# muzishen/IMAGDressing

Hardware: AMD Instinct MI355X
Metric: 512x512 50-step images/sec (whole node) (higher is better)
Workload: dtype bf16

## Files before the change

imagdressing_amd/_lib.py:

```python
from __future__ import annotations

import ctypes as C
import os

_HERE = os.path.dirname(os.path.abspath(__file__))
LIB_PATH = os.environ.get("IMD_LIB_PATH") or os.path.join(_HERE, "libimagdressing_hip.so")

ABI_VERSION = 9

u16p = C.POINTER(C.c_uint16)
f32p = C.POINTER(C.c_float)


class _Sized(C.Structure):

    def __init__(self, *args, **kw):
        super().__init__(*args, **kw)
        self.struct_bytes = C.sizeof(self)


class HeadsDest(C.Structure):
    _fields_ = [("ptr", C.c_void_p), ("kind", C.c_int), ("DP", C.c_int), ("L", C.c_int), ("scale", C.c_float)]


# ... 58 lines not shown
        ("z", C.c_void_p), ("eps", C.c_void_p), ("x_next", C.c_void_p),
        ("B", C.c_int), ("HW", C.c_int),
        ("guidance", C.c_float), ("sqrt_a_t", C.c_float), ("sqrt_1m_a_t", C.c_float),
        ("sqrt_a_prev", C.c_float), ("sqrt_1m_a_prev", C.c_float),
        ("mask", C.c_void_p), ("z_img", C.c_void_p), ("noise", C.c_void_p),
        ("sqrt_a_next", C.c_float), ("sqrt_1m_a_next", C.c_float), ("dtype", C.c_int),
        ("coefs", C.c_void_p), ("var_noise", C.c_void_p), ("sigma", C.c_float),
    ]


SYMBOLS = {
    "imd_abi_version": (C.c_int, []),
    "imd_last_error": (C.c_char_p, []),
    "imd_device_check": (C.c_int, [C.c_int]),
    "imd_conv_gemm": (C.c_int, [C.POINTER(ConvGemmParams), C.c_int, C.c_void_p]),
    "imd_conv_gemm_auto_cfg": (C.c_int, [C.c_int, C.c_int]),
    "imd_conv_gemm_auto_split": (C.c_int, [C.c_int, C.c_int, C.c_int, C.c_int]),
    "imd_attention": (C.c_int, [C.POINTER(AttnParams), C.c_void_p]),
    "imd_attention_dup_supported": (C.c_int, [C.c_int, C.c_int, C.c_int]),
    "imd_attention_phase_split_supported": (C.c_int, [C.c_int]),
    "imd_attention_fp8": (C.c_int, [C.POINTER(AttnParams), C.c_int, C.c_int, C.c_int, C.c_void_p]),
    "imd_attn_quantize_fp8": (C.c_int, [C.c_void_p, C.c_void_p, C.c_int, C.c_long, C.c_int, C.c_int, C.c_float, C.c_int, C.c_void_p]),
    "imd_set_tuning": (C.c_int, [C.c_int, C.c_int]),
    "imd_get_tuning": (C.c_int, [C.c_int]),
    "imd_attn_padded_dims": (C.c_int, [C.c_int, C.POINTER(C.c_int), C.POINTER(C.c_int)]),
    "imd_groupnorm": (C.c_int, [C.POINTER(GroupNormParams), C.c_void_p]),
    "imd_groupnorm_coeffs": (C.c_int, [C.POINTER(GroupNormParams), C.c_void_p, C.c_void_p, C.c_void_p]),
    "imd_conv_patch_supported": (C.c_int, [C.POINTER(ConvGemmParams)]),
    "imd_conv_patch2_supported": (C.c_int, [C.POINTER(ConvGemmParams)]),
    "imd_conv_patch3_supported": (C.c_int, [C.POINTER(ConvGemmParams)]),
# ... 56 lines not shown
```

imagdressing_amd/csrc/capi.cpp:

```cpp
#include <atomic>
#include <mutex>
#include <stdarg.h>
#include <stdio.h>
#include <string.h>

#include "imd_kernels.h"

namespace {
thread_local char g_err[512] = "";
}

int imd_set_error(const char* fmt, ...) {
    va_list ap;
    va_start(ap, fmt);
    vsnprintf(g_err, sizeof(g_err), fmt, ap);
    va_end(ap);
    return 1;
}

int imd_check_launch(const char* what) {
    hipError_t e = hipGetLastError();
    if (e != hipSuccess) return imd_set_error("%s: launch failed: %s", what, hipGetErrorString(e));
    return 0;
}
// ... 58 lines not shown
    IMD_REQUIRE(p != nullptr, "conv_gemm: null params");
    IMD_REQUIRE_SIZE(p, "conv_gemm");
    IMD_REQUIRE(p->x && p->w, "conv_gemm: null input/weight pointer");
    IMD_REQUIRE(p->mode == IMD_OUT_HEADS || p->out != nullptr, "conv_gemm: null output pointer");
    IMD_REQUIRE(p->Hout > 0 && p->Wout > 0 && p->Hin > 0 && p->Win > 0, "conv_gemm: bad geometry");
    IMD_REQUIRE(p->stride == 1 || p->stride == 2, "conv_gemm: stride must be 1 or 2");
    IMD_REQUIRE(p->M % (p->Hout * p->Wout) == 0, "conv_gemm: M (%d) is not a multiple of Hout*Wout (%d)", p->M, p->Hout * p->Wout);
    if (p->mode == IMD_OUT_HEADS) {
        IMD_REQUIRE(p->hC > 0 && p->hH > 0 && p->hD > 0 && p->hC == p->hH * p->hD, "conv_gemm: bad head split C=%d H=%d D=%d", p->hC, p->hH, p->hD);
        IMD_REQUIRE(p->N % p->hC == 0 && p->N / p->hC <= 3, "conv_gemm: N (%d) must be 1..3 splits of %d channels", p->N, p->hC);
        IMD_REQUIRE(p->hD % 8 == 0, "conv_gemm: head dim must be a multiple of 8");
        IMD_REQUIRE(p->act != IMD_ACT_GEGLU && !p->out_f32, "conv_gemm: head-split output excludes GEGLU / fp32 output");
    }
    if (p->act == IMD_ACT_GEGLU) IMD_REQUIRE(!p->out_f32 && !p->res, "conv_gemm: GEGLU excludes fp32 output and residual");
    return imd_launch_conv_gemm(*p, cfg, (hipStream_t)stream);
}

int imd_conv_gemm_auto_cfg(int M, int N) { return imd_conv_gemm_choose_cfg(M, N); }
int imd_conv_gemm_auto_split(int M, int N, int K, int cfg) { return imd_conv_gemm_choose_split(M, N, K, cfg < 0 ? imd_conv_gemm_choose_cfg(M, N) : cfg); }

int imd_attention(const imd_attn_params* p, void* stream) {
    IMD_REQUIRE(p != nullptr, "attention: null params");
    IMD_REQUIRE_SIZE(p, "attention");
    IMD_REQUIRE(p->q && p->k1 && p->v1t && p->out, "attention: null q/k/v/out pointer");
    IMD_REQUIRE((p->k2 == nullptr) == (p->v2t == nullptr), "attention: k2 and v2t must be given together");
    IMD_REQUIRE(p->out_ld >= p->H * p->D && p->out_ld % 4 == 0, "attention: bad out_ld %d", p->out_ld);
    return imd_launch_attention(*p, (hipStream_t)stream);
}

int imd_attention_fp8(const imd_attn_params* p, int eq, int ek, int ev, void* stream) {
// ... 193 lines not shown
```

imagdressing_amd/csrc/conv_gemm.hip:

```cpp
#include "gemm_common.h"

namespace {

template <int BM, int BN, int BK, int WAVES_M> struct TileCfg {
    static constexpr int STRIDE = BK * 2 + 16;
    static constexpr int MAIN = 2 * (BM + BN) * STRIDE;
    static constexpr int CLD = BN + 4;
    static constexpr int EROWS = BM / WAVES_M;
    static constexpr int EPI = EROWS * CLD * 4;
    static constexpr int LDS = MAIN > EPI ? MAIN : EPI;
};

template <bool F16, int BM, int BN, int BK, int WAVES_M, int WAVES_N, int DEPTH>
__global__ __launch_bounds__(WAVES_M * WAVES_N * 64, (WAVES_M * WAVES_N == 4) ? 2 : 1) void conv_gemm_kernel(const ConvGemmParams p) {
    constexpr int NT = WAVES_M * WAVES_N * 64;
    using E = El<F16>;
    using T = TileCfg<BM, BN, BK, WAVES_M>;
    constexpr int TM = BM / WAVES_M / 32;
    constexpr int TN = BN / WAVES_N / 32;
    constexpr int STRIDE = T::STRIDE;
    constexpr int VPR = BK / 8;
    constexpr int RSTEP = NT / VPR;
    constexpr int A_VECS = BM / RSTEP;
    constexpr int W_VECS = BN / RSTEP;
// ... 576 lines not shown
    if (s > 8) s = 8;
    return s < 1 ? 1 : (int)s;
}

bool imd_conv_gemm_fill_extents(ConvGemmParams& p) {
    if (p.Hout <= 0 || p.Wout <= 0 || p.M <= 0) return false;
    const size_t npix = (size_t)(p.M / (p.Hout * p.Wout)) * p.Hin * p.Win;
    if (npix == 0) return false;
    const size_t xb = ((npix - 1) * (size_t)p.x_pix_stride + p.Cin) * 2, wb = (size_t)p.N * p.K * 2;
    if (xb >= 0xffffffffull || wb >= 0xffffffffull) return false;
    p.x_bytes = (uint32_t)xb;
    p.w_bytes = (uint32_t)wb;
    return true;
}

int imd_launch_conv_gemm(const ConvGemmParams& p_in, int cfg, hipStream_t s) {
    ConvGemmParams p = p_in;
    if (p.M <= 0 || p.N <= 0 || p.K <= 0) return imd_set_error("conv_gemm: empty problem M=%d N=%d K=%d", p.M, p.N, p.K);
    if ((p.K % 8) || (p.Cin % 8) || (p.x_pix_stride % 8))
        return imd_set_error("conv_gemm: K (%d), Cin (%d) and pixel stride (%d) must be multiples of 8", p.K, p.Cin, p.x_pix_stride);
    if (p.N % 4) return imd_set_error("conv_gemm: N (%d) must be a multiple of 4", p.N);
    if (p.taps != 1 && p.taps != 9) return imd_set_error("conv_gemm: taps must be 1 or 9 (got %d)", p.taps);
    if (p.K != p.taps * p.Cin) return imd_set_error("conv_gemm: K (%d) != taps*Cin (%d)", p.K, p.taps * p.Cin);
    if (p.mode == OUT_HEADS && (p.hD % 8)) return imd_set_error("conv_gemm: head dim (%d) must be a multiple of 8", p.hD);
    if (p.act == ACT_GEGLU && (p.N % 8)) return imd_set_error("conv_gemm: GEGLU needs N %% 8 == 0");
    if (!imd_conv_gemm_fill_extents(p)) return imd_set_error("conv_gemm: operand larger than 4 GiB");
    if (cfg < 0) cfg = imd_conv_gemm_choose_cfg(p.M, p.N);
    if (p.split_k < 1) p.split_k = 1;
    const unsigned tag = (unsigned)p_in.flags & IMD_TUNING_TAG_MASK;
    if (tag != 0 && tag != (unsigned)IMD_TUNING_PER_CALL)
        return imd_set_error("conv_gemm: flags = 0x%x on entry is neither 0 nor IMD_TUNING_PER_CALL | bits (an uninitialised parameter block?)", (unsigned)p_in.flags);
// ... 31 lines not shown
                                      : (long)((p.M + bm - 1) / bm) * ((p.N + bn - 1) / bn);
        if (tiles > IMD_SPLITK_COUNTERS || (size_t)p.M * p.N * 4 >= 0x80000000ull) p.splitk_counters = nullptr;
    }
    if (p.split_k > 1) {
        if (p.mode == OUT_HEADS || p.act == ACT_GEGLU) return imd_set_error("conv_gemm: split-K supports row-major epilogues only");
        if (!p.splitk_ws) return imd_set_error("conv_gemm: split_k = %d needs a workspace", p.split_k);
    }
    if (p.dtype != IMD_DTYPE_BF16 && p.dtype != IMD_DTYPE_F16) return imd_set_error("conv_gemm: unknown dtype %d", p.dtype);
    if ((p.gn_a != nullptr) != (p.gn_b != nullptr)) return imd_set_error("conv_gemm: gn_a and gn_b must be given together");
    if (p.gn_a != nullptr && cfg != 5) return imd_set_error("conv_gemm: the fused GroupNorm prologue needs tile config 5 (got %d)", cfg);
    if (p.res_rows != 0 && cfg != 12)
        return imd_set_error("conv_gemm: a periodic residual (res_rows = %d) exists in the K = 320 row-resident projection only (tile config 12, got %d)", p.res_rows, cfg);
    if (p.gn_in_partial != nullptr && !imd_row_linear_gn_in_supported_of(p, cfg))
        return imd_set_error("conv_gemm: gn_in_* (GroupNorm of the input rows) exists in the row-resident projections only (tile configs 12 / 13 / 14 with H W a multiple of "
                             "their row block; got cfg=%d K=%d HW=%d): ask imd_row_linear_gn_in_supported() first", cfg, p.K, p.Hout * p.Wout);
    const bool h = p.dtype == IMD_DTYPE_F16;
    switch (cfg) {
        case 0: return h ? launch_cfg<true, 128, 128, 64, 2, 2>(p, s) : launch_cfg<false, 128, 128, 64, 2, 2>(p, s);
        case 1: return h ? launch_cfg<true, 128, 64, 64, 2, 2>(p, s) : launch_cfg<false, 128, 64, 64, 2, 2>(p, s);
        case 2: return h ? launch_cfg<true, 64, 64, 64, 2, 2>(p, s) : launch_cfg<false, 64, 64, 64, 2, 2>(p, s);
        case 3: return h ? launch_cfg<true, 64, 64, 64, 2, 2, 4>(p, s) : launch_cfg<false, 64, 64, 64, 2, 2, 4>(p, s);
        case 4: return h ? launch_cfg<true, 128, 128, 32, 2, 2>(p, s) : launch_cfg<false, 128, 128, 32, 2, 2>(p, s);
        case 6: return h ? launch_cfg<true, 64, 320, 32, 2, 2>(p, s) : launch_cfg<false, 64, 320, 32, 2, 2>(p, s);
        case 7: return h ? launch_cfg<true, 64, 64, 32, 2, 2, 4>(p, s) : launch_cfg<false, 64, 64, 32, 2, 2, 4>(p, s);
        case 8: return h ? launch_cfg<true, 128, 128, 32, 2, 2, 4>(p, s) : launch_cfg<false, 128, 128, 32, 2, 2, 4>(p, s);
        case 9: return h ? launch_cfg<true, 256, 128, 32, 4, 2>(p, s) : launch_cfg<false, 256, 128, 32, 4, 2>(p, s);
        case 10: return h ? launch_cfg<true, 256, 256, 32, 4, 2>(p, s) : launch_cfg<false, 256, 256, 32, 4, 2>(p, s);
        case 11: return h ? launch_cfg<true, 128, 320, 64, 4, 2>(p, s) : launch_cfg<false, 128, 320, 64, 4, 2>(p, s);
        case 5: {
            int rc = imd_launch_conv_patch(p, s);
            if (rc || p.split_k <= 1 || p.splitk_counters != nullptr) return rc;
            return launch_splitk_finish(p, s, "conv_patch split-K finish");
        }
        case 29: {
            p.splitk_counters = nullptr;
            int rc = imd_launch_conv_patch64(p, s);
            if (rc || p.split_k <= 1) return rc;
            return launch_splitk_finish(p, s, "conv_patch split-K finish");
        }
        case 21: {
            p.splitk_counters = nullptr;
            int rc = imd_launch_conv_patch2(p, s);
            if (rc || p.split_k <= 1) return rc;
            return launch_splitk_finish(p, s, "conv_patch2 split-K finish");
        }
// ... 42 lines not shown
```

imagdressing_amd/csrc/conv_patch.hip:

```cpp
#include <type_traits>

#include "gemm_common.h"
#include "lds_dma.h"

namespace {

constexpr int TH = 8, TW = 16;
constexpr int PW = TW + 2, PH = TH + 2;
constexpr int NPIX = PH * PW;
constexpr int CK = 32;
constexpr int RSTR = CK * 2 + 16;
constexpr int BN = 128;
constexpr int A_BYTES = NPIX * RSTR;
constexpr int W_BYTES = BN * RSTR;
constexpr int MAIN_LDS = 2 * A_BYTES + 2 * W_BYTES;
constexpr int CLD = BN + 4;
constexpr int EROWS = 64;
constexpr int EPI_LDS = EROWS * CLD * 4;
constexpr int PATCH_LDS = MAIN_LDS > EPI_LDS ? MAIN_LDS : EPI_LDS;
constexpr int A_VECS = (NPIX * (CK / 8) + 255) / 256;
__device__ constexpr unsigned char kColPix[32] = {0, 1, 2, 3, 8, 9, 10, 11, 12, 13, 14, 15, 4, 5, 6, 7,
                                                  30, 31, 16, 17, 22, 23, 24, 25, 26, 27, 28, 29, 18, 19, 20, 21};
constexpr int W_VECS = BN * (CK / 8) / 256;

// ... 1 lines not shown
constexpr int PATCH_DMA_LDS = 2 * AB_D + NWR_D * WB_D;
static_assert(PATCH_DMA_LDS >= EPI_LDS, "the epilogue tile must fit the main-loop LDS");
template <int CKD> struct PD {
    static constexpr int RB = CKD * 2, LPR = RB / 16;
    static constexpr int APIECES = (NPIX * RB + 1023) / 1024;
    static constexpr int APW = (APIECES + 3) / 4;
    static constexpr int AB = APW * 4 * 1024;
    static constexpr int WPW = BN * RB / 1024 / 4;
    static constexpr int WB = WPW * 4 * 1024;
    static constexpr int NWR = CKD == 32 ? 3 : 2;
    static constexpr int LDS = 2 * AB + NWR * WB;
    static_assert(LDS >= EPI_LDS, "the epilogue tile must fit the main-loop LDS");
    static __device__ __forceinline__ int swz(int r) { return CKD == 32 ? (r >> 2) & 3 : (r >> 1) & 7; }
};

template <bool F16, bool DMA, int CKD = 32>
__global__ __launch_bounds__(256, CKD == 32 ? 3 : 2) void conv3x3_patch_kernel(const ConvGemmParams p) {
    static_assert(CKD == 32 || DMA, "64-channel chunks exist for the LDS-DMA form only");
    using G = PD<CKD>;
    using E = El<F16>;
    extern __shared__ __attribute__((aligned(16))) char smem[];
    char* const Abuf = smem;
    char* const Wbuf = smem + 2 * A_BYTES;

    const int tid = threadIdx.x;
    const int lane = tid & 63;
    const int wave = tid >> 6;
    const int wm0 = (wave >> 1) * 64;
    const int wn0 = (wave & 1) * 64;
    const int hi = lane >> 5, col = lane & 31;
    const int cpix = kColPix[col];

    const int H = p.Hout, W = p.Wout;
// ... 98 lines not shown
#pragma unroll
            for (int r = 0; r < 16; ++r) acc[a][bb][r] = 0.f;

    int a_frag[2];
#pragma unroll
    for (int bb = 0; bb < 2; ++bb) {
        const int q = wm0 + bb * 32 + cpix;
        a_frag[bb] = ((q / TW) * PW + (q % TW)) * RSTR + hi * 16;
    }
    const int w_frag = (wn0 + col) * RSTR + hi * 16;
    const bool wave_live = n0 + wn0 < p.N;

    if constexpr (DMA) {
        const int wv = __builtin_amdgcn_readfirstlane(wave);
        const uint32_t smem_base = (uint32_t)(uintptr_t)smem;
        const v4i_t dx = raw_rsrc(p.x, p.x_bytes), dw = raw_rsrc(p.w, p.w_bytes);
        constexpr uint32_t FAR = 0x80000000u;
        uint32_t acur[G::APW], wcur[G::WPW];
        uint32_t adst[G::APW], wdst[G::WPW];
#pragma unroll
        for (int i = 0; i < G::APW; ++i) {
            const int slot = (wv * G::APW + i) * 64 + lane, pp = slot / G::LPR, piece = (slot % G::LPR) ^ G::swz(pp);
            acur[i] = FAR;
            if (pp < NPIX) {
                const int iy = y0 - 1 + pp / PW, ix = x0 - 1 + pp % PW;
                if ((unsigned)iy < (unsigned)H && (unsigned)ix < (unsigned)W) {
                    const int sy = p.ups ? (iy >> 1) : iy, sx = p.ups ? (ix >> 1) : ix;
                    acur[i] = (uint32_t)(((b * p.Hin + sy) * p.Win + sx) * p.x_pix_stride + piece * 8 + c_begin * CKD) * 2u;
                }
            }
            adst[i] = smem_base + (uint32_t)((wv * G::APW + i) * 1024);
        }
#pragma unroll
        for (int i = 0; i < G::WPW; ++i) {
            const int slot = (wv * G::WPW + i) * 64 + lane, row = slot / G::LPR, piece = (slot % G::LPR) ^ G::swz(row);
            wcur[i] = (n0 + row < p.N) ? (uint32_t)(((size_t)(n0 + row) * p.K + piece * 8 + c_begin * CKD) * 2) : FAR;
            wdst[i] = smem_base + (uint32_t)(2 * G::AB + (wv * G::WPW + i) * 1024);
        }
        const uint32_t w_tap = (uint32_t)(p.Cin * 2), w_chunk = (uint32_t)(CKD * 2) - 8u * w_tap;
        auto dma_patch = [&](auto buf_c) __attribute__((always_inline)) {
#pragma unroll
            for (int i = 0; i < G::APW; ++i) {
                asm volatile("s_add_u32 m0, %1, %3\n\ts_nop 0\n\tbuffer_load_dwordx4 %0, %2, 0 offen lds"
                             : : "v"(acur[i]), "s"(adst[i]), "s"(dx), "n"(decltype(buf_c)::value * G::AB) : "memory", "scc");
                acur[i] += (uint32_t)(CKD * 2);
            }
        };
        auto dma_w = [&](auto ring_c, auto cross_c) __attribute__((always_inline)) {
#pragma unroll
            for (int i = 0; i < G::WPW; ++i) {
                asm volatile("s_add_u32 m0, %1, %3\n\ts_nop 0\n\tbuffer_load_dwordx4 %0, %2, 0 offen lds"
                             : : "v"(wcur[i]), "s"(wdst[i]), "s"(dw), "n"(decltype(ring_c)::value * G::WB) : "memory", "scc");
                wcur[i] += decltype(cross_c)::value ? w_chunk : w_tap;
            }
// ... 253 lines not shown

bool imd_conv_patch_supported(const ConvGemmParams& p) {
    const bool geom = p.ups ? (p.Hout == 2 * p.Hin && p.Wout == 2 * p.Win && p.gn_a == nullptr && !(g_gemm_flags & 512))
                            : (p.Hin == p.Hout && p.Win == p.Wout);
    return p.taps == 9 && p.stride == 1 && !p.pad_br_only && geom && p.Hout >= TH && p.Wout >= TW && (p.Cin % CK) == 0 &&
           p.mode == OUT_ROWMAJOR && p.act != ACT_GEGLU;
}

bool imd_conv_patch64_supported(const ConvGemmParams& p) {
    return imd_conv_patch_supported(p) && (p.Cin % 64) == 0 && p.gn_a == nullptr && !(g_gemm_flags & 512) && p.x_bytes < 0x80000000u && p.w_bytes < 0x80000000u;
}

int imd_launch_conv_patch64(const ConvGemmParams& p, hipStream_t s) {
    if (!imd_conv_patch64_supported(p)) return imd_set_error("conv_patch (128-byte rows): unsupported problem (needs 3x3 stride 1, H >= 8, W >= 16, Cin %% 64 == 0, operands < 2 GiB, no fused GroupNorm)");
    const bool h = p.dtype == IMD_DTYPE_F16;
    typedef void (*kern_t)(const ConvGemmParams);
    const kern_t kern = h ? conv3x3_patch_kernel<true, true, 64> : conv3x3_patch_kernel<false, true, 64>;
    if (int rc_attr = imd_lds_attr(reinterpret_cast<const void*>(kern), PD<64>::LDS, "conv_patch")) return rc_attr;
    const int B = p.M / (p.Hout * p.Wout);
    const long blocks = (long)B * ((p.Hout + TH - 1) / TH) * ((p.Wout + TW - 1) / TW) * ((p.N + BN - 1) / BN);
    hipLaunchKernelGGL(kern, dim3((unsigned)blocks, (unsigned)p.split_k), dim3(256), PD<64>::LDS, s, p);
    return imd_check_launch("conv_patch (128-byte rows)");
}

int imd_launch_conv_patch(const ConvGemmParams& p, hipStream_t s) {
    if (!imd_conv_patch_supported(p)) return imd_set_error("conv_patch: unsupported geometry (needs 3x3 stride 1, H >= 8, W >= 16, Cin %% 32 == 0)");
    const bool h = p.dtype == IMD_DTYPE_F16;
    const bool dma = p.gn_a == nullptr && !(g_gemm_flags & 512) && (p.ups || (p.x_bytes < 0x80000000u && p.w_bytes < 0x80000000u));
    if (p.ups && (p.x_bytes >= 0x80000000u || p.w_bytes >= 0x80000000u)) return imd_set_error("conv_patch: fused upsample needs operands < 2 GiB");
    typedef void (*kern_t)(const ConvGemmParams);
    const kern_t kern = dma ? (h ? conv3x3_patch_kernel<true, true> : conv3x3_patch_kernel<false, true>)
                            : (h ? conv3x3_patch_kernel<true, false> : conv3x3_patch_kernel<false, false>);
    const int lds = dma ? PATCH_DMA_LDS : PATCH_LDS;
    if (int rc_attr = imd_lds_attr(reinterpret_cast<const void*>(kern), lds, "conv_patch")) return rc_attr;
    const int B = p.M / (p.Hout * p.Wout);
    const long blocks = (long)B * ((p.Hout + TH - 1) / TH) * ((p.Wout + TW - 1) / TW) * ((p.N + BN - 1) / BN);
    hipLaunchKernelGGL(kern, dim3((unsigned)blocks, (unsigned)p.split_k), dim3(256), lds, s, p);
    return imd_check_launch("conv_patch");
}
```

imagdressing_amd/csrc/imd_kernels.h:

```cpp
#pragma once
#include <hip/hip_runtime.h>
#include <stdint.h>

#include "../../include/imagdressing_hip.h"

typedef uint16_t bf16_t;
typedef imd_heads_dest HeadsDest;
typedef imd_conv_gemm_params ConvGemmParams;
typedef imd_attn_params AttnParams;
typedef imd_groupnorm_params GroupNormParams;
typedef imd_layernorm_params LayerNormParams;
typedef imd_ddim_params DdimParams;

enum { ACT_NONE = IMD_ACT_NONE, ACT_SILU = IMD_ACT_SILU, ACT_GEGLU = IMD_ACT_GEGLU, ACT_GELU = IMD_ACT_GELU, ACT_QUICK_GELU = IMD_ACT_QUICK_GELU };
enum { OUT_ROWMAJOR = IMD_OUT_ROWMAJOR, OUT_HEADS = IMD_OUT_HEADS };

int imd_set_error(const char* fmt, ...);
int imd_check_launch(const char* what);
int imd_lds_attr(const void* kern, int bytes, const char* what);
int imd_cu_count8();

int imd_conv_gemm_choose_cfg(int M, int N);
int imd_conv_gemm_choose_split(int M, int N, int K, int cfg);
int imd_launch_conv_gemm(const ConvGemmParams& p, int cfg, hipStream_t s);
bool imd_conv_gemm_fill_extents(ConvGemmParams& p);
bool imd_conv_patch_supported(const ConvGemmParams& p);
bool imd_conv_patch2_supported(const ConvGemmParams& p);
int imd_launch_conv_patch2(const ConvGemmParams& p, hipStream_t s);
bool imd_conv_patch3_supported(const ConvGemmParams& p);
int imd_launch_conv_patch3(const ConvGemmParams& p, hipStream_t s);
bool imd_conv_patch4_supported(const ConvGemmParams& p);
int imd_launch_conv_patch4(const ConvGemmParams& p, hipStream_t s);
int imd_conv_patch3_stats_parts_of(const ConvGemmParams& p, int nw);
bool imd_conv_patch64_supported(const ConvGemmParams& p);
int imd_launch_conv_patch64(const ConvGemmParams& p, hipStream_t s);
bool imd_conv_img_supported(const ConvGemmParams& p);
int imd_launch_conv_img(const ConvGemmParams& p, hipStream_t s);
int imd_conv_patch_stats_parts_of(const ConvGemmParams& p);
int imd_conv_gemm_stats_parts_of(const ConvGemmParams& p, int cfg);
bool imd_conv_gemm_gn_out_supported_of(const ConvGemmParams& p, int cfg);
bool imd_row_linear_gn_in_supported_of(const ConvGemmParams& p, int cfg);
int imd_launch_conv_patch(const ConvGemmParams& p, hipStream_t s);
bool imd_row_linear_supported(const ConvGemmParams& p);
int imd_launch_row_linear(const ConvGemmParams& p, int ln, float ln_eps, hipStream_t s);
bool imd_row_linear_k640_supported(const ConvGemmParams& p);
int imd_launch_row_linear_k640(const ConvGemmParams& p, int ln, float ln_eps, hipStream_t s);
bool imd_row_linear_k1280_supported(const ConvGemmParams& p);
int imd_launch_row_linear_k1280(const ConvGemmParams& p, int ln, float ln_eps, hipStream_t s);
bool imd_row_qkv_supported(const ConvGemmParams& p);
int imd_launch_row_qkv(const ConvGemmParams& p, int ln, float ln_eps, hipStream_t s);
bool imd_gemm_dma_supported(const ConvGemmParams& p);
int imd_launch_gemm_dma(const ConvGemmParams& p, hipStream_t s);
int imd_launch_gemm_dma128(const ConvGemmParams& p, int stages, hipStream_t s);
int imd_launch_gemm_dma256(const ConvGemmParams& p, int form, hipStream_t s);
bool imd_conv_dma_supported(const ConvGemmParams& p);
int imd_launch_ff_geglu(const imd_ff_params& p, hipStream_t s);
int imd_launch_attention(const AttnParams& p, hipStream_t s);
// ... 30 lines not shown
```

imagdressing_amd/ops.py:

```python
from __future__ import annotations

import functools
import ctypes as C
from typing import Dict, Optional, Sequence, Tuple

import torch

from . import _lib as L

ACT_NONE, ACT_SILU, ACT_GEGLU, ACT_GELU, ACT_QUICK_GELU = 0, 1, 2, 3, 4
bf16 = torch.bfloat16
f16 = torch.float16
DTYPE_CODE = {torch.bfloat16: 0, torch.float16: 1}


def _code(t: torch.Tensor, name: str = "tensor") -> int:
    try:
        return DTYPE_CODE[t.dtype]
    except KeyError:
        raise L.ImdError(f"{name}: expected a bfloat16 or float16 tensor, got {t.dtype}") from None


try:
    _raw_stream, _cur_dev = torch._C._cuda_getCurrentRawStream, torch._C._cuda_getDevice
# ... 12 lines not shown
        raise TypeError(f"{name}: expected a torch.Tensor, got {type(t)}")
    if not t.is_cuda:
        raise L.ImdError(f"{name}: tensor is on {t.device}; imagdressing_amd runs on MI355X only (no CPU path)")
    if t.dtype != dtype:
        raise L.ImdError(f"{name}: expected dtype {dtype}, got {t.dtype}")
    if not t.is_contiguous():
        raise L.ImdError(f"{name}: tensor must be contiguous")
    return t.data_ptr()


def _opt(t: Optional[torch.Tensor], dtype, name: str) -> Optional[int]:
    return None if t is None else _dev(t, dtype, name)


_checked_devices = set()


def ensure_device(device: torch.device):
    if device.type != "cuda":
        raise L.ImdError(f"tensor is on {device}; imagdressing_amd runs on MI355X (gfx950) only -- there is no CPU path")
    idx = device.index if device.index is not None else torch.cuda.current_device()
    if idx not in _checked_devices:
        L.check(L.load().imd_device_check(idx))
        _checked_devices.add(idx)


_ws: Dict[Tuple, torch.Tensor] = {}


def workspace(tag: str, shape: Sequence[int], dtype, device, init=None) -> torch.Tensor:
# ... 57 lines not shown
PATCH_CONV = True
PATCH_MIN_W = 32
SPLITK_IN_KERNEL = False
FUSED_FF = True
FUSED_FF_MIN_ROWS = 24576
import os as _os
FUSED_GN_STATS = _os.environ.get("IMD_FUSED_GN_STATS", "1") != "0"
CFG_PAIR_DEDUP = _os.environ.get("IMD_CFG_PAIR_DEDUP", "1") != "0"
FUSED_GN_CONV = _os.environ.get("IMD_FUSED_GN_CONV", "0") == "1"
FUSED_GN_FINISH = _os.environ.get("IMD_FUSED_GN_FINISH", "0") == "1"
FUSED_GN_PROJ = _os.environ.get("IMD_FUSED_GN_PROJ", "1") != "0"
FUSED_CONCAT_STATS = _os.environ.get("IMD_FUSED_CONCAT_STATS", "1") != "0"
PERIODIC_RES = _os.environ.get("IMD_PERIODIC_RES", "1") != "0"
GENERIC_GN_STATS = _os.environ.get("IMD_GENERIC_GN_STATS", "0") == "1"
TEMB_TABLE = _os.environ.get("IMD_TEMB_TABLE", "1") != "0"
FUSED_GN_PROJ_CFGS = tuple(int(c) for c in _os.environ.get("IMD_FUSED_GN_PROJ_CFGS", "12,13,14").split(",") if c)
CFG_PAIR_ATTN = _os.environ.get("IMD_CFG_PAIR_ATTN", "1") != "0"
FUSED_LN = True
GEMM_TRACE = None
GEMM_EVENT_HOOK = None
_GEMM_TABLE = None
_CFG_DECISIONS: Dict[Tuple, Tuple[int, int]] = {}

TUNING_PER_CALL = 0x5A000000
ATTN_VARIANT_MAX = 13


import contextvars

_TUNING = contextvars.ContextVar("imd_tuning_scope", default=None)
# ... 47 lines not shown
                _GEMM_TABLE = json.load(f).get("shapes", {})
        except FileNotFoundError:
            _GEMM_TABLE = {}
    return _GEMM_TABLE


def conv_gemm(
    x: torch.Tensor, w: torch.Tensor, *, M: int, N: int, Cin: int, taps: int = 1,
    Hin: int = 1, Win: int = 1, Hout: int = 1, Wout: int = 1, stride: int = 1, ups: bool = False,
    x_pix_stride: Optional[int] = None, out: Optional[torch.Tensor] = None, out_ld: Optional[int] = None,
    bias: Optional[torch.Tensor] = None, rowvec: Optional[torch.Tensor] = None, rowvec_stride: int = 0,
    rowvec_off: int = 0, res: Optional[torch.Tensor] = None, res_ld: Optional[int] = None, out_scale: float = 1.0,
    act: int = ACT_NONE, out_f32: bool = False,
    heads: Optional[dict] = None, cfg: int = -1, split_k: int = 0,
    gn: Optional[tuple] = None, pad_br_only: bool = False, ln_eps: Optional[float] = None, gn_stats_groups: int = 0,
    gn_out: Optional[tuple] = None, gn_in: Optional[tuple] = None,
) -> Optional[torch.Tensor]:
    ensure_device(x.device)
    K = taps * Cin
    p = L.ConvGemmParams()
    p.flags = _gemm_call_flags()
    dt = x.dtype
    p.dtype = _code(x, "x")
    p.x = _dev(x, dt, "x")
    p.w = _dev(w, dt, "w")
    if w.numel() != N * K:
        raise L.ImdError(f"conv_gemm: weight has {w.numel()} elements, expected N*K = {N}*{K}")
    p.M, p.N, p.K = M, N, K
    p.Cin, p.taps, p.Hin, p.Win, p.Hout, p.Wout, p.stride, p.ups = Cin, taps, Hin, Win, Hout, Wout, stride, int(ups)
    p.x_pix_stride = Cin if x_pix_stride is None else x_pix_stride
    p.bias = _opt(bias, torch.float32, "bias")
# ... 131 lines not shown
            out._imd_gn_applied = True
            return out
        p.gn_out_gamma = p.gn_out_beta = None
        p.gn_out_groups = 0
    stats = None
    if gn_stats_groups and FUSED_GN_STATS and heads is None and not out_f32 and act != ACT_GEGLU and \
            (cfg in (5, 22, 23, 29) or split_k > 1 or (GENERIC_GN_STATS and cfg in (-1, 0, 1, 2, 3, 4, 7))):
        p.gn_stats_groups = gn_stats_groups
        nparts = lib.imd_conv_gemm_stats_parts(C.byref(p), cfg)
        if nparts > 0:
            Bimg = M // (Hout * Wout)
            stats = (torch.empty((Bimg, nparts, gn_stats_groups, 2), dtype=torch.float32, device=x.device), nparts, gn_stats_groups)
            p.gn_stats_out = stats[0].data_ptr()
        else:
            p.gn_stats_groups = 0
    if GEMM_EVENT_HOOK is not None:
        e0, e1 = torch.cuda.Event(enable_timing=True), torch.cuda.Event(enable_timing=True)
        e0.record()
        L.check(lib.imd_conv_gemm(C.byref(p), cfg, _stream()))
        e1.record()
        GEMM_EVENT_HOOK.setdefault((f"{M},{N},{K},{taps},{stride},{int(ups)}|{Hout}x{Wout}", cfg, split_k), []).append((e0, e1))
    else:
        L.check(lib.imd_conv_gemm(C.byref(p), cfg, _stream()))
    if stats is not None:
        out._imd_gn_stats = stats
    return out


_splitk_ws: Dict[Tuple, torch.Tensor] = {}


_splitk_cnt: Dict[Tuple, torch.Tensor] = {}


def splitk_counters(device) -> torch.Tensor:
    key = (str(device), _stream())
    t = _splitk_cnt.get(key)
    if t is None:
# ... 55 lines not shown
    ensure_device(x2d.device)
    M, C_ = x2d.shape
    dt = x2d.dtype
    if out is None:
        out = torch.empty((M, C_), dtype=dt, device=x2d.device)
    p = L.FfParams()
    p.x, p.w1, p.b1 = _dev(x2d, dt, "x"), _dev(packed["w1"], dt, "w1"), _dev(packed["b1"], torch.float32, "b1")
    p.w2, p.b2, p.out = _dev(packed["w2"], dt, "w2"), _dev(packed["b2"], torch.float32, "b2"), _dev(out, dt, "out")
    p.M, p.C, p.inner, p.x_ld, p.out_ld = M, packed["C"], packed["inner"], x2d.stride(0), out.stride(0)
    p.ln, p.ln_eps, p.dtype = int(packed["ln"]), float(ln_eps), _code(x2d, "x")
    _count("gemm_conv", 2.0 * M * packed["C"] * 2 * packed["inner"] + 2.0 * M * packed["inner"] * packed["C"])
    L.check(L.load().imd_ff_geglu(C.byref(p), _stream()))
    return out


def conv2d_nhwc(x: torch.Tensor, w: torch.Tensor, bias=None, *, taps=9, stride=1, ups=False, rowvec=None,
                rowvec_stride=0, rowvec_off=0, res=None, out_scale=1.0, act=ACT_NONE, out_f32=False, cfg=-1, split_k=0, gn=None,
                pad_br_only=False, gn_stats_groups=0, gn_out=None, gn_in=None) -> torch.Tensor:
    B, H, W, Cin = x.shape
    Cout = w.shape[0]
    Hl, Wl = (2 * H, 2 * W) if ups else (H, W)
    Ho, Wo = ((Hl + stride - 1) // stride, (Wl + stride - 1) // stride)
    M = B * Ho * Wo
    out = conv_gemm(x, w, M=M, N=Cout, Cin=Cin, taps=taps, Hin=H, Win=W, Hout=Ho, Wout=Wo, stride=stride, ups=ups,
                    bias=bias, rowvec=rowvec, rowvec_stride=rowvec_stride, rowvec_off=rowvec_off, res=res, out_scale=out_scale, act=act,
                    out_f32=out_f32, cfg=cfg, split_k=split_k, gn=gn, pad_br_only=pad_br_only, gn_stats_groups=gn_stats_groups, gn_out=gn_out, gn_in=gn_in)
    r = out.view(B, Ho, Wo, -1)
    if getattr(out, "_imd_gn_applied", False):
        r._imd_gn_applied = True
    st = getattr(out, "_imd_gn_stats", None)
    if st is not None:
        r._imd_gn_stats = st
    return r


ATTN_EVENT_HOOK = None


FUSED_OUT_PROJ = _os.environ.get("IMD_FUSED_OUT_PROJ", "0") == "1"


# ... 354 lines not shown
```

imagdressing_amd/unet.py:

```python
from __future__ import annotations

import math
from types import SimpleNamespace
from typing import Dict, List, Optional

import torch

from . import ops
from .hub import PretrainedMixin

FUSED_LN_CHANNELS = (320, 640, 1280)

bf16 = torch.bfloat16

SD15_CONFIG = dict(
    in_channels=4, out_channels=4, block_out_channels=(320, 640, 1280, 1280), layers_per_block=2,
    attention_head_dim=8, cross_attention_dim=768, norm_num_groups=32, sample_size=64,
    down_attn=(True, True, True, False), time_cond_proj_dim=None,
)


def _resnet_shapes(p, cin, cout, temb):
    s = {f"{p}.norm1.weight": (cin,), f"{p}.norm1.bias": (cin,),
         f"{p}.conv1.weight": (cout, cin, 3, 3), f"{p}.conv1.bias": (cout,),
# ... 131 lines not shown

class ConvOp:

    def __init__(self, weight: torch.Tensor, bias: Optional[torch.Tensor], device, dtype=bf16):
        cout, cin, kh, kw = weight.shape
        assert (kh, kw) in ((1, 1), (3, 3))
        cin_p = (cin + 7) // 8 * 8
        w = weight.detach().to(device=device, dtype=torch.float32).permute(0, 2, 3, 1)
        if cin_p != cin:
            w = torch.nn.functional.pad(w, (0, cin_p - cin))
        cout_p = (cout + 3) // 4 * 4
        self.weight = w.reshape(cout, kh * kw * cin_p).to(dtype).contiguous()
        self.bias = None if bias is None else _f32(bias, device)
        self.cin, self.cin_p, self.cout, self.taps = cin, cin_p, cout, kh * kw
        assert cout_p == cout, "output channels must be a multiple of 4"

    def __call__(self, x, **kw):
        return ops.conv2d_nhwc(x, self.weight, self.bias, taps=self.taps, **kw)


class NormParams:
    def __init__(self, sd, prefix, device):
        self.weight = _f32(sd[prefix + ".weight"], device)
        self.bias = _f32(sd[prefix + ".bias"], device)


class _Identity:
    def __call__(self, x):
        return x


class Attention:

# ... 462 lines not shown
```

include/imagdressing_hip.h:

```cpp
#ifndef IMAGDRESSING_HIP_H
#define IMAGDRESSING_HIP_H

#include <stdint.h>

#ifdef __cplusplus
extern "C" {
#endif

#define IMD_ABI_VERSION 9

enum { IMD_ACT_NONE = 0, IMD_ACT_SILU = 1, IMD_ACT_GEGLU = 2, IMD_ACT_GELU = 3, IMD_ACT_QUICK_GELU = 4  };
enum { IMD_OUT_ROWMAJOR = 0, IMD_OUT_HEADS = 1 };
enum { IMD_DTYPE_BF16 = 0, IMD_DTYPE_F16 = 1 };

typedef struct imd_heads_dest {
    uint16_t* ptr;
    int kind;
    int DP;
    int L;
    float scale;
} imd_heads_dest;

#define IMD_TUNING_PER_CALL 0x5A000000
#define IMD_TUNING_TAG_MASK 0xFF000000u
// ... 115 lines not shown
    const float* mask;
    const float* z_img;
    const float* noise;
    float sqrt_a_next, sqrt_1m_a_next;
    int dtype;
    const float* coefs;
    const float* var_noise;
    float sigma;
} imd_ddim_params;

int imd_abi_version(void);
const char* imd_last_error(void);
int imd_device_check(int device);

int imd_conv_gemm(const imd_conv_gemm_params* p, int cfg, void* stream);
int imd_conv_gemm_auto_cfg(int M, int N);
int imd_conv_gemm_auto_split(int M, int N, int K, int cfg);

int imd_attention(const imd_attn_params* p, void* stream);
int imd_attention_fp8(const imd_attn_params* p, int eq, int ek, int ev, void* stream);
int imd_attn_quantize_fp8(const uint16_t* src, uint8_t* dst, int kind, long count, int LP, int exp2_scale, float pad_val, int dtype,
                          void* stream);
int imd_row_linear_gn_in_supported(const imd_conv_gemm_params* p, int cfg);
int imd_conv_gemm_gn_out_supported(const imd_conv_gemm_params* p);
int imd_attention_dup_supported(int H, int N, int D);
int imd_attention_phase_split_supported(int D);
int imd_attn_padded_dims(int D, int* dpk, int* dpv);
int imd_set_tuning(int knob, int value);
int imd_get_tuning(int knob);

// ... 43 lines not shown
```

Baseline: 6.977.

## Feed 3x3 patch conv from a tile-contiguous pre-swizzled weight copy

Adds a packed weight layout for the LDS-DMA 3x3 patch convolution. Each 128-output tile and 32-channel chunk is stored as contiguous 8 KB blocks with the LDS swizzle already applied, so the weight DMA reads whole contiguous lines instead of strided rows. The packed copy is built lazily per conv layer and cached by weight version. It is skipped during graph capture and used only when the grid fills the device. The cost is extra weight memory and a one-time pack per layer.

```diff
diff --git a/imagdressing_amd/_lib.py b/imagdressing_amd/_lib.py
--- a/imagdressing_amd/_lib.py
+++ b/imagdressing_amd/_lib.py
@@ -96,6 +96,8 @@
     "imd_last_error": (C.c_char_p, []),
     "imd_device_check": (C.c_int, [C.c_int]),
     "imd_conv_gemm": (C.c_int, [C.POINTER(ConvGemmParams), C.c_int, C.c_void_p]),
+    "imd_conv_patch_tiled": (C.c_int, [C.POINTER(ConvGemmParams), C.c_void_p, C.c_size_t, C.c_void_p]),
+    "imd_conv_patch_tiled_bytes": (C.c_size_t, [C.c_int, C.c_int]),
     "imd_conv_gemm_auto_cfg": (C.c_int, [C.c_int, C.c_int]),
     "imd_conv_gemm_auto_split": (C.c_int, [C.c_int, C.c_int, C.c_int, C.c_int]),
     "imd_attention": (C.c_int, [C.POINTER(AttnParams), C.c_void_p]),
diff --git a/imagdressing_amd/csrc/capi.cpp b/imagdressing_amd/csrc/capi.cpp
--- a/imagdressing_amd/csrc/capi.cpp
+++ b/imagdressing_amd/csrc/capi.cpp
@@ -96,6 +96,18 @@
     }
     if (p->act == IMD_ACT_GEGLU) IMD_REQUIRE(!p->out_f32 && !p->res, "conv_gemm: GEGLU excludes fp32 output and residual");
     return imd_launch_conv_gemm(*p, cfg, (hipStream_t)stream);
+}
+
+size_t imd_conv_patch_tiled_bytes(int N, int Cin) { return imd_conv_patch_tiled_bytes_of(N, Cin); }
+
+int imd_conv_patch_tiled(const imd_conv_gemm_params* p, const void* w_tiled, size_t w_tiled_bytes, void* stream) {
+    IMD_REQUIRE(p != nullptr, "conv_patch_tiled: null params");
+    IMD_REQUIRE_SIZE(p, "conv_patch_tiled");
+    IMD_REQUIRE(p->x && w_tiled, "conv_patch_tiled: null input / tiled weight pointer");
+    IMD_REQUIRE(p->mode == IMD_OUT_ROWMAJOR && p->out != nullptr, "conv_patch_tiled: needs a row-major output");
+    IMD_REQUIRE(p->Hout > 0 && p->Wout > 0 && p->Hin > 0 && p->Win > 0, "conv_patch_tiled: bad geometry");
+    IMD_REQUIRE(p->M % (p->Hout * p->Wout) == 0, "conv_patch_tiled: M (%d) is not a multiple of Hout*Wout (%d)", p->M, p->Hout * p->Wout);
+    return imd_launch_conv_gemm(*p, 5, (hipStream_t)stream, w_tiled, w_tiled_bytes);
 }
 
 int imd_conv_gemm_auto_cfg(int M, int N) { return imd_conv_gemm_choose_cfg(M, N); }
diff --git a/imagdressing_amd/csrc/conv_gemm.hip b/imagdressing_amd/csrc/conv_gemm.hip
--- a/imagdressing_amd/csrc/conv_gemm.hip
+++ b/imagdressing_amd/csrc/conv_gemm.hip
@@ -614,7 +614,7 @@
     return true;
 }
 
-int imd_launch_conv_gemm(const ConvGemmParams& p_in, int cfg, hipStream_t s) {
+int imd_launch_conv_gemm(const ConvGemmParams& p_in, int cfg, hipStream_t s, const void* w_tiled, size_t w_tiled_bytes) {
     ConvGemmParams p = p_in;
     if (p.M <= 0 || p.N <= 0 || p.K <= 0) return imd_set_error("conv_gemm: empty problem M=%d N=%d K=%d", p.M, p.N, p.K);
     if ((p.K % 8) || (p.Cin % 8) || (p.x_pix_stride % 8))
@@ -676,6 +676,7 @@
     if (p.gn_in_partial != nullptr && !imd_row_linear_gn_in_supported_of(p, cfg))
         return imd_set_error("conv_gemm: gn_in_* (GroupNorm of the input rows) exists in the row-resident projections only (tile configs 12 / 13 / 14 with H W a multiple of "
                              "their row block; got cfg=%d K=%d HW=%d): ask imd_row_linear_gn_in_supported() first", cfg, p.K, p.Hout * p.Wout);
+    if (w_tiled != nullptr && cfg != 5) return imd_set_error("conv_gemm: the tile-contiguous weight copy belongs to tile config 5 (got %d)", cfg);
     const bool h = p.dtype == IMD_DTYPE_F16;
     switch (cfg) {
         case 0: return h ? launch_cfg<true, 128, 128, 64, 2, 2>(p, s) : launch_cfg<false, 128, 128, 64, 2, 2>(p, s);
@@ -690,7 +691,7 @@
         case 10: return h ? launch_cfg<true, 256, 256, 32, 4, 2>(p, s) : launch_cfg<false, 256, 256, 32, 4, 2>(p, s);
         case 11: return h ? launch_cfg<true, 128, 320, 64, 4, 2>(p, s) : launch_cfg<false, 128, 320, 64, 4, 2>(p, s);
         case 5: {
-            int rc = imd_launch_conv_patch(p, s);
+            int rc = w_tiled != nullptr ? imd_launch_conv_patch_tiled(p, w_tiled, w_tiled_bytes, s) : imd_launch_conv_patch(p, s);
             if (rc || p.split_k <= 1 || p.splitk_counters != nullptr) return rc;
             return launch_splitk_finish(p, s, "conv_patch split-K finish");
         }
diff --git a/imagdressing_amd/csrc/conv_patch.hip b/imagdressing_amd/csrc/conv_patch.hip
--- a/imagdressing_amd/csrc/conv_patch.hip
+++ b/imagdressing_amd/csrc/conv_patch.hip
@@ -39,9 +39,10 @@
     static __device__ __forceinline__ int swz(int r) { return CKD == 32 ? (r >> 2) & 3 : (r >> 1) & 7; }
 };
 
-template <bool F16, bool DMA, int CKD = 32>
-__global__ __launch_bounds__(256, CKD == 32 ? 3 : 2) void conv3x3_patch_kernel(const ConvGemmParams p) {
+template <bool F16, bool DMA, int CKD = 32, bool TILED = false>
+__global__ __launch_bounds__(256, CKD == 32 ? 3 : 2) void conv3x3_patch_kernel(const ConvGemmParams p, const void* wt, uint32_t wt_bytes) {
     static_assert(CKD == 32 || DMA, "64-channel chunks exist for the LDS-DMA form only");
+    static_assert(!TILED || (DMA && CKD == 32), "the tile-contiguous weight source exists for the LDS-DMA form with 32-channel chunks only");
     using G = PD<CKD>;
     using E = El<F16>;
     extern __shared__ __attribute__((aligned(16))) char smem[];
@@ -170,7 +171,7 @@
     if constexpr (DMA) {
         const int wv = __builtin_amdgcn_readfirstlane(wave);
         const uint32_t smem_base = (uint32_t)(uintptr_t)smem;
-        const v4i_t dx = raw_rsrc(p.x, p.x_bytes), dw = raw_rsrc(p.w, p.w_bytes);
+        const v4i_t dx = raw_rsrc(p.x, p.x_bytes), dw = TILED ? raw_rsrc(wt, wt_bytes) : raw_rsrc(p.w, p.w_bytes);
         constexpr uint32_t FAR = 0x80000000u;
         uint32_t acur[G::APW], wcur[G::WPW];
         uint32_t adst[G::APW], wdst[G::WPW];
@@ -190,10 +191,13 @@
 #pragma unroll
         for (int i = 0; i < G::WPW; ++i) {
             const int slot = (wv * G::WPW + i) * 64 + lane, row = slot / G::LPR, piece = (slot % G::LPR) ^ G::swz(row);
-            wcur[i] = (n0 + row < p.N) ? (uint32_t)(((size_t)(n0 + row) * p.K + piece * 8 + c_begin * CKD) * 2) : FAR;
+            if (TILED)
+                wcur[i] = (n0 + row < p.N) ? (uint32_t)((tile_n * nchunks + c_begin) * 9) * (uint32_t)G::WB + (uint32_t)slot * 16u : FAR;
+            else
+                wcur[i] = (n0 + row < p.N) ? (uint32_t)(((size_t)(n0 + row) * p.K + piece * 8 + c_begin * CKD) * 2) : FAR;
             wdst[i] = smem_base + (uint32_t)(2 * G::AB + (wv * G::WPW + i) * 1024);
         }
-        const uint32_t w_tap = (uint32_t)(p.Cin * 2), w_chunk = (uint32_t)(CKD * 2) - 8u * w_tap;
+        const uint32_t w_tap = TILED ? (uint32_t)G::WB : (uint32_t)(p.Cin * 2), w_chunk = TILED ? (uint32_t)G::WB : (uint32_t)(CKD * 2) - 8u * w_tap;
         auto dma_patch = [&](auto buf_c) __attribute__((always_inline)) {
 #pragma unroll
             for (int i = 0; i < G::APW; ++i) {
@@ -477,12 +481,12 @@
 int imd_launch_conv_patch64(const ConvGemmParams& p, hipStream_t s) {
     if (!imd_conv_patch64_supported(p)) return imd_set_error("conv_patch (128-byte rows): unsupported problem (needs 3x3 stride 1, H >= 8, W >= 16, Cin %% 64 == 0, operands < 2 GiB, no fused GroupNorm)");
     const bool h = p.dtype == IMD_DTYPE_F16;
-    typedef void (*kern_t)(const ConvGemmParams);
+    typedef void (*kern_t)(const ConvGemmParams, const void*, uint32_t);
     const kern_t kern = h ? conv3x3_patch_kernel<true, true, 64> : conv3x3_patch_kernel<false, true, 64>;
     if (int rc_attr = imd_lds_attr(reinterpret_cast<const void*>(kern), PD<64>::LDS, "conv_patch")) return rc_attr;
     const int B = p.M / (p.Hout * p.Wout);
     const long blocks = (long)B * ((p.Hout + TH - 1) / TH) * ((p.Wout + TW - 1) / TW) * ((p.N + BN - 1) / BN);
-    hipLaunchKernelGGL(kern, dim3((unsigned)blocks, (unsigned)p.split_k), dim3(256), PD<64>::LDS, s, p);
+    hipLaunchKernelGGL(kern, dim3((unsigned)blocks, (unsigned)p.split_k), dim3(256), PD<64>::LDS, s, p, (const void*)nullptr, 0u);
     return imd_check_launch("conv_patch (128-byte rows)");
 }
 
@@ -491,13 +495,36 @@
     const bool h = p.dtype == IMD_DTYPE_F16;
     const bool dma = p.gn_a == nullptr && !(g_gemm_flags & 512) && (p.ups || (p.x_bytes < 0x80000000u && p.w_bytes < 0x80000000u));
     if (p.ups && (p.x_bytes >= 0x80000000u || p.w_bytes >= 0x80000000u)) return imd_set_error("conv_patch: fused upsample needs operands < 2 GiB");
-    typedef void (*kern_t)(const ConvGemmParams);
+    typedef void (*kern_t)(const ConvGemmParams, const void*, uint32_t);
     const kern_t kern = dma ? (h ? conv3x3_patch_kernel<true, true> : conv3x3_patch_kernel<false, true>)
                             : (h ? conv3x3_patch_kernel<true, false> : conv3x3_patch_kernel<false, false>);
     const int lds = dma ? PATCH_DMA_LDS : PATCH_LDS;
     if (int rc_attr = imd_lds_attr(reinterpret_cast<const void*>(kern), lds, "conv_patch")) return rc_attr;
     const int B = p.M / (p.Hout * p.Wout);
     const long blocks = (long)B * ((p.Hout + TH - 1) / TH) * ((p.Wout + TW - 1) / TW) * ((p.N + BN - 1) / BN);
-    hipLaunchKernelGGL(kern, dim3((unsigned)blocks, (unsigned)p.split_k), dim3(256), lds, s, p);
+    hipLaunchKernelGGL(kern, dim3((unsigned)blocks, (unsigned)p.split_k), dim3(256), lds, s, p, (const void*)nullptr, 0u);
     return imd_check_launch("conv_patch");
 }
+
+size_t imd_conv_patch_tiled_bytes_of(int N, int Cin) {
+    if (N <= 0 || Cin <= 0 || (Cin % CK) != 0) return 0;
+    return (size_t)((N + BN - 1) / BN) * (size_t)(Cin / CK) * 9 * PD<32>::WB;
+}
+
+int imd_launch_conv_patch_tiled(const ConvGemmParams& p, const void* wt, size_t wt_bytes, hipStream_t s) {
+    if (!imd_conv_patch_supported(p)) return imd_set_error("conv_patch (tiled weights): unsupported geometry (needs 3x3 stride 1, H >= 8, W >= 16, Cin %% 32 == 0)");
+    if (p.gn_a != nullptr || (g_gemm_flags & 512))
+        return imd_set_error("conv_patch (tiled weights): the tile-contiguous weight copy feeds the LDS-DMA form only (no fused GroupNorm prologue, knob 2 bit 9 clear)");
+    if (wt == nullptr || wt_bytes != imd_conv_patch_tiled_bytes_of(p.N, p.Cin))
+        return imd_set_error("conv_patch (tiled weights): the copy is %zu bytes, N = %d and Cin = %d need %zu", wt_bytes, p.N, p.Cin, imd_conv_patch_tiled_bytes_of(p.N, p.Cin));
+    if (((uintptr_t)wt & 127) != 0) return imd_set_error("conv_patch (tiled weights): the copy must start on a 128-byte boundary (every 8 KB block = 64 whole L2 lines)");
+    if (p.x_bytes >= 0x80000000u || wt_bytes >= 0x80000000ull) return imd_set_error("conv_patch (tiled weights): operands must be < 2 GiB");
+    const bool h = p.dtype == IMD_DTYPE_F16;
+    typedef void (*kern_t)(const ConvGemmParams, const void*, uint32_t);
+    const kern_t kern = h ? conv3x3_patch_kernel<true, true, 32, true> : conv3x3_patch_kernel<false, true, 32, true>;
+    if (int rc_attr = imd_lds_attr(reinterpret_cast<const void*>(kern), PATCH_DMA_LDS, "conv_patch")) return rc_attr;
+    const int B = p.M / (p.Hout * p.Wout);
+    const long blocks = (long)B * ((p.Hout + TH - 1) / TH) * ((p.Wout + TW - 1) / TW) * ((p.N + BN - 1) / BN);
+    hipLaunchKernelGGL(kern, dim3((unsigned)blocks, (unsigned)p.split_k), dim3(256), PATCH_DMA_LDS, s, p, wt, (uint32_t)wt_bytes);
+    return imd_check_launch("conv_patch (tiled weights)");
+}
diff --git a/imagdressing_amd/csrc/imd_kernels.h b/imagdressing_amd/csrc/imd_kernels.h
--- a/imagdressing_amd/csrc/imd_kernels.h
+++ b/imagdressing_amd/csrc/imd_kernels.h
@@ -22,7 +22,7 @@
 
 int imd_conv_gemm_choose_cfg(int M, int N);
 int imd_conv_gemm_choose_split(int M, int N, int K, int cfg);
-int imd_launch_conv_gemm(const ConvGemmParams& p, int cfg, hipStream_t s);
+int imd_launch_conv_gemm(const ConvGemmParams& p, int cfg, hipStream_t s, const void* w_tiled = nullptr, size_t w_tiled_bytes = 0);
 bool imd_conv_gemm_fill_extents(ConvGemmParams& p);
 bool imd_conv_patch_supported(const ConvGemmParams& p);
 bool imd_conv_patch2_supported(const ConvGemmParams& p);
@@ -41,6 +41,8 @@
 bool imd_conv_gemm_gn_out_supported_of(const ConvGemmParams& p, int cfg);
 bool imd_row_linear_gn_in_supported_of(const ConvGemmParams& p, int cfg);
 int imd_launch_conv_patch(const ConvGemmParams& p, hipStream_t s);
+size_t imd_conv_patch_tiled_bytes_of(int N, int Cin);
+int imd_launch_conv_patch_tiled(const ConvGemmParams& p, const void* wt, size_t wt_bytes, hipStream_t s);
 bool imd_row_linear_supported(const ConvGemmParams& p);
 int imd_launch_row_linear(const ConvGemmParams& p, int ln, float ln_eps, hipStream_t s);
 bool imd_row_linear_k640_supported(const ConvGemmParams& p);
diff --git a/imagdressing_amd/ops.py b/imagdressing_amd/ops.py
--- a/imagdressing_amd/ops.py
+++ b/imagdressing_amd/ops.py
@@ -50,6 +50,11 @@
 
 
 _checked_devices = set()
+
+
+@functools.lru_cache(maxsize=None)
+def _cu_count(device: torch.device) -> int:
+    return torch.cuda.get_device_properties(device).multi_processor_count
 
 
 def ensure_device(device: torch.device):
@@ -137,6 +142,7 @@
 PERIODIC_RES = _os.environ.get("IMD_PERIODIC_RES", "1") != "0"
 GENERIC_GN_STATS = _os.environ.get("IMD_GENERIC_GN_STATS", "0") == "1"
 TEMB_TABLE = _os.environ.get("IMD_TEMB_TABLE", "1") != "0"
+CONV_TILED_W = _os.environ.get("IMD_CONV_TILED_W", "1") != "0"
 FUSED_GN_PROJ_CFGS = tuple(int(c) for c in _os.environ.get("IMD_FUSED_GN_PROJ_CFGS", "12,13,14").split(",") if c)
 CFG_PAIR_ATTN = _os.environ.get("IMD_CFG_PAIR_ATTN", "1") != "0"
 FUSED_LN = True
@@ -214,7 +220,7 @@
     act: int = ACT_NONE, out_f32: bool = False,
     heads: Optional[dict] = None, cfg: int = -1, split_k: int = 0,
     gn: Optional[tuple] = None, pad_br_only: bool = False, ln_eps: Optional[float] = None, gn_stats_groups: int = 0,
-    gn_out: Optional[tuple] = None, gn_in: Optional[tuple] = None,
+    gn_out: Optional[tuple] = None, gn_in: Optional[tuple] = None, w_tiled=None,
 ) -> Optional[torch.Tensor]:
     ensure_device(x.device)
     K = taps * Cin
@@ -376,14 +382,28 @@
             p.gn_stats_out = stats[0].data_ptr()
         else:
             p.gn_stats_groups = 0
+    wt = None
+    if w_tiled is not None and CONV_TILED_W and cfg == 5 and gn is None and not (lib.imd_get_tuning(2) & 512):
+        if not callable(w_tiled):
+            wt = w_tiled
+        elif (M // (Hout * Wout)) * ((Hout + 7) // 8) * ((Wout + 15) // 16) * ((N + 127) // 128) * split_k >= _cu_count(x.device):
+            wt = w_tiled()
+        if wt is not None and (wt.dtype != dt or wt.device != x.device or not wt.is_contiguous()):
+            raise L.ImdError(f"conv_gemm: the tiled weight copy is {wt.dtype} on {wt.device}, the input {dt} on {x.device}")
+
+    def launch():
+        if wt is not None:
+            L.check(lib.imd_conv_patch_tiled(C.byref(p), wt.data_ptr(), wt.numel() * wt.element_size(), _stream()))
+        else:
+            L.check(lib.imd_conv_gemm(C.byref(p), cfg, _stream()))
     if GEMM_EVENT_HOOK is not None:
         e0, e1 = torch.cuda.Event(enable_timing=True), torch.cuda.Event(enable_timing=True)
         e0.record()
-        L.check(lib.imd_conv_gemm(C.byref(p), cfg, _stream()))
+        launch()
         e1.record()
         GEMM_EVENT_HOOK.setdefault((f"{M},{N},{K},{taps},{stride},{int(ups)}|{Hout}x{Wout}", cfg, split_k), []).append((e0, e1))
     else:
-        L.check(lib.imd_conv_gemm(C.byref(p), cfg, _stream()))
+        launch()
     if stats is not None:
         out._imd_gn_stats = stats
     return out
@@ -469,9 +489,26 @@
     return out
 
 
+def conv_w_tiled_bytes(N: int, Cin: int) -> int:
+    return 0 if Cin <= 0 or Cin % 32 else (N + 127) // 128 * (Cin // 32) * 9 * 8192
+
+
+def pack_conv_w_tiled(w: torch.Tensor, N: int, Cin: int) -> torch.Tensor:
+    if w.numel() != N * 9 * Cin or Cin % 32 or w.element_size() != 2:
+        raise L.ImdError(f"pack_conv_w_tiled: expected a 16-bit [N = {N}][9 * Cin = {9 * Cin}] weight with Cin % 32 == 0, got {tuple(w.shape)} {w.dtype}")
+    nt, nch = (N + 127) // 128, Cin // 32
+    wp = w.reshape(N, 9 * Cin)
+    if nt * 128 != N:
+        wp = torch.cat([wp, wp.new_zeros((nt * 128 - N, 9 * Cin))])
+    t = wp.view(nt, 128, 9, nch, 4, 8).permute(0, 3, 2, 1, 4, 5)
+    r = torch.arange(128, device=w.device)
+    src = torch.arange(4, device=w.device)[None, :] ^ ((r >> 2) & 3)[:, None]
+    return t[:, :, :, r[:, None], src, :].contiguous().view(-1)
+
+
 def conv2d_nhwc(x: torch.Tensor, w: torch.Tensor, bias=None, *, taps=9, stride=1, ups=False, rowvec=None,
                 rowvec_stride=0, rowvec_off=0, res=None, out_scale=1.0, act=ACT_NONE, out_f32=False, cfg=-1, split_k=0, gn=None,
-                pad_br_only=False, gn_stats_groups=0, gn_out=None, gn_in=None) -> torch.Tensor:
+                pad_br_only=False, gn_stats_groups=0, gn_out=None, gn_in=None, w_tiled=None) -> torch.Tensor:
     B, H, W, Cin = x.shape
     Cout = w.shape[0]
     Hl, Wl = (2 * H, 2 * W) if ups else (H, W)
@@ -479,7 +516,8 @@
     M = B * Ho * Wo
     out = conv_gemm(x, w, M=M, N=Cout, Cin=Cin, taps=taps, Hin=H, Win=W, Hout=Ho, Wout=Wo, stride=stride, ups=ups,
                     bias=bias, rowvec=rowvec, rowvec_stride=rowvec_stride, rowvec_off=rowvec_off, res=res, out_scale=out_scale, act=act,
-                    out_f32=out_f32, cfg=cfg, split_k=split_k, gn=gn, pad_br_only=pad_br_only, gn_stats_groups=gn_stats_groups, gn_out=gn_out, gn_in=gn_in)
+                    out_f32=out_f32, cfg=cfg, split_k=split_k, gn=gn, pad_br_only=pad_br_only, gn_stats_groups=gn_stats_groups, gn_out=gn_out, gn_in=gn_in,
+                    w_tiled=w_tiled)
     r = out.view(B, Ho, Wo, -1)
     if getattr(out, "_imd_gn_applied", False):
         r._imd_gn_applied = True
diff --git a/imagdressing_amd/unet.py b/imagdressing_amd/unet.py
--- a/imagdressing_amd/unet.py
+++ b/imagdressing_amd/unet.py
@@ -169,9 +169,21 @@
         self.bias = None if bias is None else _f32(bias, device)
         self.cin, self.cin_p, self.cout, self.taps = cin, cin_p, cout, kh * kw
         assert cout_p == cout, "output channels must be a multiple of 4"
+        self._tiled = None
+
+    def tiled_weight(self):
+        w = self.weight
+        t = self._tiled
+        if t is not None and t[0] is w and t[1] == w._version:
+            return t[2]
+        if self.taps != 9 or self.cin_p % 32 or (w.is_cuda and torch.cuda.is_current_stream_capturing()):
+            return None
+        wt = ops.pack_conv_w_tiled(w, self.cout, self.cin_p)
+        self._tiled = (w, w._version, wt)
+        return wt
 
     def __call__(self, x, **kw):
-        return ops.conv2d_nhwc(x, self.weight, self.bias, taps=self.taps, **kw)
+        return ops.conv2d_nhwc(x, self.weight, self.bias, taps=self.taps, w_tiled=self.tiled_weight, **kw)
 
 
 class NormParams:
diff --git a/include/imagdressing_hip.h b/include/imagdressing_hip.h
--- a/include/imagdressing_hip.h
+++ b/include/imagdressing_hip.h
@@ -1,6 +1,7 @@
 #ifndef IMAGDRESSING_HIP_H
 #define IMAGDRESSING_HIP_H
 
+#include <stddef.h>
 #include <stdint.h>
 
 #ifdef __cplusplus
@@ -153,6 +154,8 @@
 int imd_device_check(int device);
 
 int imd_conv_gemm(const imd_conv_gemm_params* p, int cfg, void* stream);
+int imd_conv_patch_tiled(const imd_conv_gemm_params* p, const void* w_tiled, size_t w_tiled_bytes, void* stream);
+size_t imd_conv_patch_tiled_bytes(int N, int Cin);
 int imd_conv_gemm_auto_cfg(int M, int N);
 int imd_conv_gemm_auto_split(int M, int N, int K, int cfg);
 
```

New measurement: 7.040 (median of 6 runs). Within noise of the previous version (+0.9%).
